# GiulioRomualdi/paper_romualdi_2022_icra_centroidal-mpc-walking

Hardware: AMD Instinct MI355X
Metric: centroidal-MPC solves/sec (batch, horizon=20) (higher is better)
Workload: dtype f32

## Files before the change

paper_romualdi_2022_icra_centroidal-mpc-walking_amd/csrc/cmpc_solver.hip:

```cpp
#include "cmpc_device.h"
#include "cmpc_launch.h"

#include <cstdlib>
#include <type_traits>
#include <map>
#include <mutex>

#define NS CMPC_NS
#define NF CMPC_NF
#define NQ CMPC_NQ
#define NU CMPC_NU
#define NXA CMPC_NXA
#define NI CMPC_NI
#define PLD 39
#define GLD 30
#define RLD 36
#define NPAN 46
#define GEO 36
#define SQ_TILE_WAVES 6
#define SQ_SPIN_MAX (1 << 20)
#define SQ_PUB_FLOATS (10 * NPAN * 4 + 128 * 4)
#define ZLD 36
#define MSET (NU * RLD + NPAN * RLD + NS * 16)
#define NTRI 256
// ... 1693 lines not shown
            if (ln < NU) Pann[(NPAN - 1) * RLD + ln] = (float)res;
            else if (ln < NU + NS) qsn[ln - NU] = res;
        } else {
            const bool two = wv == 3;
            v4f acc2 = {0.f, 0.f, 0.f, 0.f};
            CPROF(2);
#pragma unroll
            for (int b = 0; b < 8; b += 2) {
                float a0, b0, a1, b1;
                if (b == 6 && sk8 && sk9) {
                    need(7);
                    operands(6, a0, b0);
                    acc = __builtin_amdgcn_mfma_f32_16x16x4f32(a0, b0, acc, 0, 0, 0);
                    if (two) acc2 = __builtin_amdgcn_mfma_f32_16x16x4f32(a0, -a0, acc2, 0, 0, 0);
                    need(8);
                    operands(7, a1, b1);
                    acc = __builtin_amdgcn_mfma_f32_16x16x4f32(a1, b1, acc, 0, 0, 0);
                    if (two) acc2 = __builtin_amdgcn_mfma_f32_16x16x4f32(a1, -a1, acc2, 0, 0, 0);
                    continue;
                }
                need(b + 2);
                operands(b, a0, b0);
                operands(b + 1, a1, b1);
                acc = __builtin_amdgcn_mfma_f32_16x16x4f32(a0, b0, acc, 0, 0, 0);
                if (two) acc2 = __builtin_amdgcn_mfma_f32_16x16x4f32(a0, -a0, acc2, 0, 0, 0);
                acc = __builtin_amdgcn_mfma_f32_16x16x4f32(a1, b1, acc, 0, 0, 0);
                if (two) acc2 = __builtin_amdgcn_mfma_f32_16x16x4f32(a1, -a1, acc2, 0, 0, 0);
                if (b == 0) {
                    gaveup = !lds_wait_ge(c.flag + 3, SQ_TILE_WAVES * (ord + 1)) || gaveup;
                    acc += v4f{Mn[pl.d0], Mn[pl.d1], Mn[pl.d2], Mn[pl.d3]};
                    if (two) acc2 += v4f{Mn[pl.ri[5]], Mn[pl.ri[6]], Mn[pl.ri[7]], Mn[pl.ri[8]]};
                }
            }
            CPROF(3);
            if (!sk8 && !sk9) {
                float a0, b0, a1, b1;
                need(9);
                operands(8, a0, b0);
                acc = __builtin_amdgcn_mfma_f32_16x16x4f32(a0, b0, acc, 0, 0, 0);
                if (two) acc2 = __builtin_amdgcn_mfma_f32_16x16x4f32(a0, -a0, acc2, 0, 0, 0);
                need(10);
                operands(9, a1, b1);
                acc = __builtin_amdgcn_mfma_f32_16x16x4f32(a1, b1, acc, 0, 0, 0);
                if (two) acc2 = __builtin_amdgcn_mfma_f32_16x16x4f32(a1, -a1, acc2, 0, 0, 0);
            } else if (!sk8 || !sk9) {
                const int b = sk8 ? 9 : 8;
                need(b + 1);
                float a0, b0;
                operands(b, a0, b0);
                acc = __builtin_amdgcn_mfma_f32_16x16x4f32(a0, b0, acc, 0, 0, 0);
                if (two) acc2 = __builtin_amdgcn_mfma_f32_16x16x4f32(a0, -a0, acc2, 0, 0, 0);
            }
            CPROF2(4);
            {
                const float r0 = acc[0], r1 = acc[1], r2 = acc[2], r3 = acc[3];
                Mn[pl.d0] = r0; Mn[pl.d1] = r1; Mn[pl.d2] = r2; Mn[pl.d3] = r3;
                if (wv == 2 || wv == 4) { Mn[pl.ri[9]] = r0; Mn[pl.ri[10]] = r1; Mn[pl.ri[11]] = r2; Mn[pl.ri[12]] = r3; }
            }
            if (two) {
                const float r0 = acc2[0], r1 = acc2[1], r2 = acc2[2], r3 = acc2[3];
                Mn[pl.ri[5]] = r0; Mn[pl.ri[6]] = r1; Mn[pl.ri[7]] = r2; Mn[pl.ri[8]] = r3;
                Mn[pl.ri[9]] = r0; Mn[pl.ri[10]] = r1; Mn[pl.ri[11]] = r2; Mn[pl.ri[12]] = r3;
            }
        }
        CPROF(4);
    }
    if (gaveup && ln == 0) sq_give_up(c);
}
template <int NT, int NC, bool FG>
__device__ __attribute__((noinline)) void sq_consume_loop(lds_t lds, int Nrt, float* fg_base, int k0_in, bool exact_in, float reg, float cmu)
{
    CMPC_PHASE_PROLOGUE;
    const int k0 = __builtin_amdgcn_readfirstlane(k0_in);
    const bool use_exact = __builtin_amdgcn_readfirstlane((int)exact_in) != 0;
    ConsPlan pl;
    cons_plan_build(pl, c, prm, tid >> 6, tid & 63, c.Brow + ((N - 1) & 1) * DSET_I);
    sq_consume_stage(c, prm, pl, tid, N, N, N - 1, -1, 0, false, use_exact, reg, cmu);
    __syncthreads();
    int ord = 0;
#pragma unroll 1
    for (int k = N - 1; k >= k0; --k) {
        ++ord;
        if (k > k0) sq_consume_stage(c, prm, pl, tid, N, k, k - 1, k - 2 >= k0 ? k - 2 : -1, ord, true, use_exact, reg, cmu);
        __syncthreads();
    }
}
template <int NT, int NC, bool FG>
__device__ __attribute__((noinline)) void sq_init(lds_t lds, int Nrt, float* fg_base, int k0_in, bool exact_in, float cmu)
{
    CMPC_PHASE_PROLOGUE;
    const int k0 = __builtin_amdgcn_readfirstlane(k0_in);
    const bool use_exact = __builtin_amdgcn_readfirstlane((int)exact_in) != 0;
    {
        float* QN = c.Qb + (N & 1) * MSET;
        double* qN = (N & 1) ? c.qs1 : c.qs;
        if (tid < NS * 16) QN[tid] = (tid >> 4) == (tid & 15) ? qdiag(prm, N, tid & 15) : 0.f;
        else if (tid >= 256 && tid < 256 + NS) qN[tid - 256] = grad_track(c, prm, N, tid - 256);
        if (tid < 4) c.flag[tid] = 0;
        if (tid >= 128 && tid < 256) c.prog[tid - 128] = 0;
        if (tid >= 256 && tid < 256 + LATE_B * NLATE) {
            const int e = tid - 256, b = e / NLATE, r = e % NLATE;
            *reinterpret_cast<float4*>(c.ZT + (NPAN * b + NS + LATE_M0 + r) * 4) = make_float4(0.f, 0.f, 0.f, 0.f);
        }
    }
    if (tid >= 256) {
        const int kd = tid >= 384 ? N - 1 : N - 2;
        if (kd >= k0) {
            use_desc_set(c, kd & 1);
            stage_desc_body(c, prm, desc_pack_t(tid & 127), kd, use_exact, cmu);
        }
    }
    __syncthreads();
}
template <int NT, int NC, bool FG>
__device__ inline int riccati_backward_sq(lds_t lds, const Ctx& c, float* fg_base, bool use_exact, float reg, float cmu, int k0)
{
    const int N = c.N;
    sq_init<NT, NC, FG>(lds, N, fg_base, k0, use_exact, cmu);
    if (threadIdx.x < 64) sq_factor_loop<NT, NC, FG>(lds, N, fg_base, k0);
    else sq_consume_loop<NT, NC, FG>(lds, N, fg_base, k0, use_exact, reg, cmu);
    return (c.flag[0] ? 1 : 0) | (c.flag[1] ? 2 : 0);
}

template <int NT, int NC, bool FG>
__device__ int riccati_backward(lds_t lds, const Ctx& c, const CmpcConsts& prm, int tid, float* fg_base, bool use_exact, float reg, float cmu, int k0 = 0)
{
    if constexpr (!FG) return riccati_backward_sq<NT, NC, FG>(lds, c, fg_base, use_exact, reg, cmu, k0);
    const int N = c.N;
    for (int e = tid; e < NXA * PLD; e += NT) c.P0[e] = 0.f;
    if (tid == 0) *c.flag = 0;
    __syncthreads();
    if (tid < NS) {
        c.P0[tid * PLD + tid] = qdiag(prm, N, tid);
        c.pv[tid] = grad_track(c, prm, N, tid);
    } else if (tid < NXA) c.pv[tid] = 0.0;
    if (tid >= 128) stage_desc<NT, NC, FG>(lds, N, fg_base, N - 1, use_exact, cmu);
    __syncthreads();
    int tpk, tqp;
    {
        const int id0 = tid, id1 = tid + 128;
        tpk = (id0 < 135 ? c.tri[id0 / 3] : 0) | ((id1 < 135 ? c.tri[id1 / 3] : 0) << 16);
        const int tq = tid - 128, tile = tid;
        tqp = ((tq >= 0 && tq < 120) ? c.tri[tq] : 0) | ((tile < 210 ? c.tri[tile] : 0) << 16);
    }
    stage_pre<NT, NC, FG>(lds, N, fg_base, N - 1, false, use_exact, reg, cmu, tpk);
    for (int k = N - 1; k >= k0; --k) {
        if (((~__builtin_amdgcn_readfirstlane(c.qmask[k])) & 63) == 63) stage_mid<NT, NC, FG, true>(lds, N, fg_base, k, use_exact, cmu, tqp);
        else stage_mid<NT, NC, FG, false>(lds, N, fg_base, k, use_exact, cmu, tqp);
        if (k > k0 || k0 == 0) stage_post_pre<NT, NC, FG>(lds, N, fg_base, k, use_exact, reg, cmu, tpk, tqp);
    }
    return *c.flag ? 1 : 0;
}

template <int UNR, bool G>
__device__ __forceinline__ void forward_sweep(const Ctx& c, const CmpcConsts& prm, int tid, int k0)
{
    const int N = c.N;
    const int r = tid & 31, half = tid >> 5, blk = r >> 2;
    float* xb = c.ybuf;
    float* yb = c.ybuf + 40;
    float* trash = c.ybuf + 72;
    unsigned yoff[20], uoff[4];
#pragma unroll
    for (int t = 0; t < 20; ++t) {
        if (half == 0) yoff[t] = t < 16 ? wt_idx(t, r) : ub_row(t - 16) + r;
        else {
            const int m = 4 + t;
            yoff[t] = blk >= (m >> 2) ? ub_row(m) + r - 4 * (m >> 2) : REC_ZERO;
        }
    }
#pragma unroll
    for (int t = 0; t < 4; ++t) {
        const int q4 = 4 * half + t;
        uoff[t] = q4 >= blk ? ub_row(r) + 4 * (q4 - blk) : REC_ZERO;
    }
    const bool corner = tid < NF;
    const int ga = corner ? tid >> 3 : 0, cj = corner ? tid & 7 : 0;
    const int ga1 = (ga + 1) % 3, ga2 = (ga + 2) % 3;
    const int j = tid < NS ? tid : 0;
    const int ja = j % 3, ja1 = (ja + 1) % 3, ja2 = (ja + 2) % 3, jct = j >= 12 ? 1 : 0;
    const int je = j < 3 ? j + 3 : 0;
    const float ce = j < 3 ? prm.dt : 0.f;
    const float cD = (j >= 3 && j < 6) ? 1.f : 0.f, cH = (j >= 6 && j < 9) ? 1.f : 0.f;
    const float posm = j >= 9 ? 1.f : 0.f;
    const float cDm0 = ja == 0 ? cD : 0.f, cDm1 = ja == 1 ? cD : 0.f, cDm2 = ja == 2 ? cD : 0.f;
    const float cHm0 = ja == 0 ? cH : 0.f, cHm1 = ja == 1 ? cH : 0.f, cHm2 = ja == 2 ? cH : 0.f;
    const float gdtm = corner ? prm.dt : 0.f, gsel = cj >= 4 ? 1.f : 0.f, jsel = jct ? 1.f : 0.f;
    const float Dm = prm.D[r % 3];
    const float dtc = prm.dt;
    if (tid < 40) xb[tid] = tid == 15 ? 1.f : 0.f;
    if (tid < NS) c.dS[NS * k0 + tid] = 0.f;
    wave_lds_sync();
    ldsf_t yp[20];
    ldsf_t upp[4];
    if (!G) {
#pragma unroll
        for (int t = 0; t < 20; ++t) yp[t] = lds_opaque(c.Lf + (size_t)REC_N * k0 + yoff[t]);
#pragma unroll
        for (int t = 0; t < 4; ++t) upp[t] = lds_opaque(c.Lf + (size_t)REC_N * k0 + uoff[t]);
    }
    ldsf_t gr1 = lds_opaque(c.geoA + GEO * k0 + 3 * cj + ga1);
    ldsf_t gr2 = lds_opaque(c.geoA + GEO * k0 + 3 * cj + ga2);
    ldsf_t gf1 = lds_opaque(c.geoA + GEO * k0 + 24 + ja1);
    ldsf_t gf2 = lds_opaque(c.geoA + GEO * k0 + 24 + ja2);
    ldsf_t gm0 = lds_opaque(c.sp + c.L.pGam(0) + k0);
    ldsf_t gm1 = lds_opaque(c.sp + c.L.pGam(1) + k0);
    ldsf_t rp = lds_opaque(c.sp + c.L.pR(jct) + 9 * k0 + ja);
    ldsf_t dp = lds_opaque(c.d + NS * k0 + j);
    ldsf_t du0p = lds_opaque(c.dU + NU * k0 + 3 * cj + ga);
    ldsf_t du1p = lds_opaque(c.dU + NU * k0 + 3 * cj + ga1);
    ldsf_t du2p = lds_opaque(c.dU + NU * k0 + 3 * cj + ga2);
    ldsf_t dqp = lds_opaque(c.dU + NU * k0 + 24 + 3 * jct);
    ldsw_t dUs = lds_opaque_w(tid < NU ? c.dU + NU * k0 + tid : trash + (tid & 7));
    const int dUst = tid < NU ? NU : 0;
    ldsw_t dSs = lds_opaque_w(tid < NS ? c.dS + NS * (k0 + 1) + tid : trash + 8 + (tid & 7));
    const int dSst = tid < NS ? NS : 0;
    ldsw_t xbs = lds_opaque_w(tid < NS ? xb + tid : trash + 16 + (tid & 3));
    ldsw_t xps = lds_opaque_w(tid < NF ? xb + 16 + tid : trash + 20 + (tid & 3));
    ldsw_t ybs = lds_opaque_w(yb + r);
    ldsf_t xsp = lds_opaque(xb + j), xep = lds_opaque(xb + je), x1p = lds_opaque(xb + ja1), x2p = lds_opaque(xb + ja2);
    ldsf_t xvp = lds_opaque(xb + 20 * half), yvp = lds_opaque(yb + 16 * half);
    PROF2_DECL;
    float ymn[20];
    auto fetch = [&](int k) {
        const RecRef<G> rec(c.Lf, N, k);
#pragma unroll
        for (int t = 0; t < 20; ++t) ymn[t] = rec.ld(yoff[t]);
    };
    if (G) fetch(k0);
    auto stage = [&](int i, int k) {
        float ym[20];
        float4 um[4];
        if (G) {
            {
                const RecRef<G> rec(c.Lf, N, k);
#pragma unroll
                for (int t = 0; t < 4; ++t) um[t] = rec.ld4(uoff[t]);
            }
#pragma unroll
            for (int t = 0; t < 20; ++t) ym[t] = ymn[t];
            fetch(k + 1 < N ? k + 1 : k);
        } else {
#pragma unroll
            for (int t = 0; t < 20; ++t) ym[t] = yp[t][REC_N * i];
#pragma unroll
            for (int t = 0; t < 4; ++t) um[t] = lds_ld4(upp[t] + REC_N * i);
        }
        const float g_r1 = gr1[GEO * i], g_r2 = gr2[GEO * i];
        const float F01 = gf1[GEO * i], F11 = gf1[GEO * i + 3], F02 = gf2[GEO * i], F12 = gf2[GEO * i + 3];
        const float gam0 = gm0[i], gam1 = gm1[i];
        const float R0 = rp[9 * i], R1 = rp[9 * i + 3], R2 = rp[9 * i + 6];
        const float dk = dp[NS * i];
        const float dgam = gam1 - gam0;
        const float g_dt = gdtm * fmaf(gsel, dgam, gam0);
        const float gamj = fmaf(jsel, dgam, gam0);
        PROF2(20);
        float4 xv[5];
#pragma unroll
        for (int t = 0; t < 5; ++t) xv[t] = lds_ld4(xvp + 4 * t);
        float ya, yc;
        {
            v2f yp = v2f{ym[0], ym[1]} * v2f{xv[0].x, xv[0].y}, yq = v2f{ym[2], ym[3]} * v2f{xv[0].z, xv[0].w};
#pragma unroll
            for (int t = 1; t < 5; ++t) {
                yp = __builtin_elementwise_fma(v2f{ym[4 * t], ym[4 * t + 1]}, v2f{xv[t].x, xv[t].y}, yp);
                yq = __builtin_elementwise_fma(v2f{ym[4 * t + 2], ym[4 * t + 3]}, v2f{xv[t].z, xv[t].w}, yq);
            }
            yp += yq;
            ya = yp[0]; yc = yp[1];
        }
        const float y = half_sum(ya + yc);
        *ybs = y;
        wave_lds_sync();
        PROF2(21);
        float4 yv[4];
        if (G) {
#pragma unroll
            for (int q = 0; q < 4; ++q) yv[q] = lds_ld4(yvp + 4 * q);
        } else lds_ld4x4(yvp, yv);
        float wsum;
        {
            v2f wp = v2f{um[0].x, um[0].y} * v2f{yv[0].x, yv[0].y}, wq = v2f{um[0].z, um[0].w} * v2f{yv[0].z, yv[0].w};
#pragma unroll
            for (int q = 1; q < 4; ++q) {
                wp = __builtin_elementwise_fma(v2f{um[q].x, um[q].y}, v2f{yv[q].x, yv[q].y}, wp);
                wq = __builtin_elementwise_fma(v2f{um[q].z, um[q].w}, v2f{yv[q].z, yv[q].w}, wq);
            }
            wp += wq;
            wsum = wp[0] + wp[1];
        }
        const float du = -half_sum(wsum);
        *dUs = du;
        dUs += dUst;
        wave_lds_sync();
        PROF2(22);
        const float u0 = du0p[NU * i], u1 = du1p[NU * i], u2 = du2p[NU * i];
        const float xs = *xsp, xe = *xep;
        const float c1 = x1p[0], c2 = x2p[0];
        const float p01 = x1p[9], p02 = x2p[9], p11 = x1p[12], p12 = x2p[12];
        const float q0 = dqp[NU * i], q1 = dqp[NU * i + 1], q2 = dqp[NU * i + 2];
        const float tD = oct_sum(g_dt * u0);
        const float tH = oct_sum(g_dt * (g_r1 * u2 - g_r2 * u1));
        const float sDH = cDm0 * readlane_f(tD, 0) + cDm1 * readlane_f(tD, 8) + cDm2 * readlane_f(tD, 16)
                          + cHm0 * readlane_f(tH, 0) + cHm1 * readlane_f(tH, 8) + cHm2 * readlane_f(tH, 16);
        const float cross = gam0 * ((p01 - c1) * F02 - (p02 - c2) * F01) + gam1 * ((p11 - c1) * F12 - (p12 - c2) * F11);
        const float land = R0 * q0 + R1 * q1 + R2 * q2;
        const float out = fmaf(posm, gamj - 1.f, 1.f) * xs + ce * xe + sDH + cH * dtc * cross + dk + posm * (1.f - gamj) * land;
        wave_lds_sync();
        *dSs = out;
        dSs += dSst;
        *xbs = out;
        *xps = -Dm * du;
        wave_lds_sync();
        PROF2(23);
    };
    auto bump = [&](int n) {
        if (!G) {
#pragma unroll
            for (int t = 0; t < 20; ++t) yp[t] += REC_N * n;
#pragma unroll
            for (int t = 0; t < 4; ++t) upp[t] += REC_N * n;
#pragma unroll
            for (int t = 0; t < 20; ++t) asm volatile("" : "+v"(yp[t]));
#pragma unroll
            for (int t = 0; t < 4; ++t) asm volatile("" : "+v"(upp[t]));
        }
        gr1 += GEO * n; gr2 += GEO * n; gf1 += GEO * n; gf2 += GEO * n; gm0 += n; gm1 += n; rp += 9 * n; dp += NS * n;
        du0p += NU * n; du1p += NU * n; du2p += NU * n; dqp += NU * n;
    };
    int k = k0;
#pragma unroll 1
    for (; k + UNR <= N; k += UNR) {
#pragma unroll
        for (int i = 0; i < UNR; ++i) stage(i, k + i);
        bump(UNR);
    }
#pragma unroll 1
    for (; k < N; ++k) {
        stage(0, k);
        bump(1);
    }
}
template <int NT, int UNR, bool G, int PART = 0>
__device__ void riccati_forward(const Ctx& c, const CmpcConsts& prm, int tid, bool affine, int k0)
{
    const int N = c.N;
    if (PART != 2 && tid < 64) forward_sweep<UNR, G>(c, prm, tid, k0);
    if (PART == 1) return;
    __syncthreads();
    for (int e = tid + NI * k0; e < N * NI; e += NT) {
        const int k = e / NI, i = e % NI;
        float dt_ = 0.f, dz_ = 0.f;
        if (row_active(c, k, i)) {
            const float t = c.T[e], z = c.Z[e];
            const float cmu = affine ? 0.f : c.dZ[e];
            const float r = row_val(c, prm, k, i, c.U + NU * k) + t;
            dt_ = -r - row_dot(c, prm, k, i, c.dU + NU * k);
            dz_ = (cmu - z * t) / t - (z / t) * dt_;
        }
        c.dT[e] = dt_; c.dZ[e] = dz_;
    }
    __syncthreads();
}

template <int UNR, bool G>
__device__ __forceinline__ void delta_sweep(const Ctx& c, const CmpcConsts& prm, int tid)
{
    const int N = c.N;
    const int r = tid & 31, half = tid >> 5, blk = r >> 2;
    float* gb = c.ybuf;
    float* lb = c.ybuf + 32;
    float* trash = c.ybuf + 72;
    unsigned loff[16], foff[8];
#pragma unroll
// ... 260 lines not shown
    const float t1 = readlane_f(v, 16), t2 = readlane_f(v, 32), t3 = readlane_f(v, 48);
    const int row = lane >> 4;
    return v + (row == 0 ? t1 + (t2 + t3) : (row == 1 ? t2 + t3 : (row == 2 ? t3 : 0.f)));
}
__device__ inline float suffix_lin(float g, float b, int lane)
{
#define CMPC_LIN_STEP(CT) { const float gn = dpp_keep<CT>(1.f, g), bn = dpp_f<CT>(b); b = fmaf(g, bn, b); g *= gn; }
    CMPC_LIN_STEP(0x101) CMPC_LIN_STEP(0x102) CMPC_LIN_STEP(0x104) CMPC_LIN_STEP(0x108)
#undef CMPC_LIN_STEP
    const int row = lane >> 4;
    const float v48 = readlane_f(b, 48);
    if (row == 2) b = fmaf(g, v48, b);
    const float v32 = readlane_f(b, 32);
    if (row == 1) b = fmaf(g, v32, b);
    const float v16 = readlane_f(b, 16);
    if (row == 0) b = fmaf(g, v16, b);
    return b;
}
__device__ __forceinline__ float costate_com_b(float w, float err, float egm, float dtm, float dF1, float dF2, float lo1, float lo2, float vh1, float vh2, float g1,
                                               float g2)
{
    float b = w * err;
    b += egm * (dF2 * lo1 - dF1 * lo2);
    b += dtm * (vh1 * g2 - vh2 * g1);
    return b;
}
__device__ __forceinline__ float costate_foot_b(float w, float err, float egm, float dtm, float gam, float dF1, float dF2, float lo1, float lo2, float vh1, float vh2,
                                                float g1, float g2)
{
    float b = w * err;
    b += egm * (dF1 * lo2 - dF2 * lo1);
    b -= dtm * gam * (vh1 * g2 - vh2 * g1);
    return b;
}
__device__ __forceinline__ float sel3(const float (&v)[3], int i) { return i == 0 ? v[0] : (i == 1 ? v[1] : v[2]); }
__device__ inline void costate_scan_axis(const Ctx& c, const CmpcConsts& prm, int lane, int ax, bool use_exact, float* vout)
{
    const int N = c.N;
    const bool valid = lane <= N, dyn = lane < N;
    const int k = valid ? lane : N, kd = dyn ? lane : N - 1;
    const int a1 = ax == 2 ? 0 : ax + 1, a2 = ax == 0 ? 2 : ax - 1;
    const float* S = c.S + NS * k;
    const float* dS = c.dS + NS * k;
    const float* geo = c.geoA + GEO * kd;
    const float* du = c.dU + NU * kd;
    const float* lo = c.LAM + NS * (kd + 1) + 6;
    const float dtm = dyn ? prm.dt : 0.f;
    const float egm = use_exact ? dtm : 0.f;
    const float on = valid ? 1.f : 0.f;
    const float gam0 = gam_of(c, 0, kd), gam1 = gam_of(c, 1, kd);
    float dF1[3], dF2[3];
    dF1[0] = gam0 * (du[a1] + du[3 + a1] + du[6 + a1] + du[9 + a1]);
    dF1[1] = gam1 * (du[12 + a1] + du[15 + a1] + du[18 + a1] + du[21 + a1]);
    dF1[2] = dF1[0] + dF1[1];
    dF2[0] = gam0 * (du[a2] + du[3 + a2] + du[6 + a2] + du[9 + a2]);
    dF2[1] = gam1 * (du[12 + a2] + du[15 + a2] + du[18 + a2] + du[21 + a2]);
    dF2[2] = dF2[0] + dF2[1];
    const float lo1 = lo[a1], lo2 = lo[a2];
    float vh[3], vhn[3];
#pragma unroll
    for (int a = 0; a < 3; ++a) {
        const float b = on * (2.f * prm.w_h) * ((S[6 + a] - c.sp[c.L.pHref() + a + 3 * k]) + dS[6 + a]);
        vh[a] = suffix_sum(b, lane);
    }
#pragma unroll
    for (int a = 0; a < 3; ++a) vhn[a] = lane_next(vh[a], lane);
    const float vh1 = sel3(vhn, a1), vh2 = sel3(vhn, a2);
    const float w = ax == 0 ? 2.f * prm.w_com0 : (ax == 1 ? 2.f * prm.w_com1 : prm.wz2[k]);
    const float bc = costate_com_b(w, (S[ax] - c.sp[c.L.pComref() + ax + 3 * k]) + dS[ax], egm, dtm, dF1[2], dF2[2], lo1, lo2, vh1, vh2, geo[30 + a1], geo[30 + a2]);
    const float vc = suffix_sum(on * bc, lane);
    float vf[2];
#pragma unroll
    for (int ct = 0; ct < 2; ++ct) {
        const float gam = ct ? gam1 : gam0;
        const int j = 9 + 3 * ct + ax;
        const float b = costate_foot_b(2.f * prm.w_pos, (S[j] - c.sp[c.L.pNom(ct) + ax + 3 * k]) + dS[j], egm, dtm, gam, dF1[ct], dF2[ct], lo1, lo2, vh1, vh2,
                                       geo[24 + 3 * ct + a1], geo[24 + 3 * ct + a2]);
        vf[ct] = suffix_lin(dyn ? gam : 1.f, on * b, lane);
    }
    const float vv = suffix_sum(dtm * lane_next(vc, lane), lane);
    if (valid && lane > 0) {
        float* o = vout + NS * k + ax;
        o[0] = vc; o[3] = vv; o[6] = sel3(vh, ax); o[9] = vf[0]; o[12] = vf[1];
    }
}
template <bool DEFER>
__device__ inline void costate_scan(const Ctx& c, const CmpcConsts& prm, int lane, float ap, bool use_exact, float* vout)
{
    const int N = c.N;
    const bool valid = lane <= N, dyn = lane < N;
    const int k = valid ? lane : N, kd = dyn ? lane : N - 1;
    const float* S = c.S + NS * k;
    const float* dS = c.dS + NS * k;
    const float* geo = c.geoA + GEO * kd;
    const float* dF = c.d + NS * kd;
    const float dtm = dyn ? prm.dt : 0.f;
    const float egm = use_exact ? dtm : 0.f;
    const float on = valid ? 1.f : 0.f;
    float lo[3];
#pragma unroll
    for (int a = 0; a < 3; ++a) lo[a] = c.LAM[NS * (kd + 1) + 6 + a];
    float lold[NS];
    if (!DEFER) {
#pragma unroll
        for (int j = 0; j < NS; ++j) lold[j] = c.LAM[NS * k + j];
    }
    float v[NS];
    float vh1[3];
#pragma unroll
    for (int a = 0; a < 3; ++a) {
        const float b = on * (2.f * prm.w_h) * ((S[6 + a] - c.sp[c.L.pHref() + a + 3 * k]) + dS[6 + a]);
        v[6 + a] = suffix_sum(b, lane);
    }
#pragma unroll
    for (int a = 0; a < 3; ++a) vh1[a] = lane_next(v[6 + a], lane);
#pragma unroll
    for (int a = 0; a < 3; ++a) {
        const int a1 = (a + 1) % 3, a2 = (a + 2) % 3;
        const float w = a == 0 ? 2.f * prm.w_com0 : (a == 1 ? 2.f * prm.w_com1 : prm.wz2[k]);
        const float b = costate_com_b(w, (S[a] - c.sp[c.L.pComref() + a + 3 * k]) + dS[a], egm, dtm, dF[6 + a1], dF[6 + a2], lo[a1], lo[a2], vh1[a1], vh1[a2],
                                      geo[30 + a1], geo[30 + a2]);
        v[a] = suffix_sum(on * b, lane);
    }
#pragma unroll
    for (int ct = 0; ct < 2; ++ct) {
        const float gam = c.sp[c.L.pGam(ct) + kd];
#pragma unroll
        for (int a = 0; a < 3; ++a) {
            const int a1 = (a + 1) % 3, a2 = (a + 2) % 3, j = 9 + 3 * ct + a;
            const float b = costate_foot_b(2.f * prm.w_pos, (S[j] - c.sp[c.L.pNom(ct) + a + 3 * k]) + dS[j], egm, dtm, gam, dF[3 * ct + a1], dF[3 * ct + a2], lo[a1],
                                           lo[a2], vh1[a1], vh1[a2], geo[24 + 3 * ct + a1], geo[24 + 3 * ct + a2]);
            v[j] = suffix_lin(dyn ? gam : 1.f, on * b, lane);
        }
    }
#pragma unroll
    for (int a = 0; a < 3; ++a) v[3 + a] = suffix_sum(dtm * lane_next(v[a], lane), lane);
    if (valid && lane > 0) {
#pragma unroll
        for (int j = 0; j < NS; ++j) {
            if (DEFER) vout[NS * k + j] = v[j];
            else c.LAM[NS * k + j] = lold[j] + ap * (v[j] - lold[j]);
        }
    }
}

__device__ void costate_update(const Ctx& c, const CmpcConsts& prm, int tid, float ap, bool use_exact)
{
    costate_force_sums(c, tid, blockDim.x);
    __syncthreads();
    if (tid < 64) costate_scan<false>(c, prm, tid, ap, use_exact, nullptr);
    __syncthreads();
}

template <int NT, int NC, bool FG, int PART>
__device__ __attribute__((noinline)) void phase_forward_part(lds_t lds, int Nrt, float* fg_base, bool affine_in)
{
    CMPC_PHASE_PROLOGUE;
    const bool affine = __builtin_amdgcn_readfirstlane((int)affine_in) != 0;
    riccati_forward<NT, NC == 0 ? 1 : (FG ? 2 : SWEEP_UNROLL), FG, PART>(c, prm, tid, affine, 0);
}
template <int NT, int NC, bool FG>
__device__ __forceinline__ void phase_forward_sweep(lds_t lds, int Nrt, float* fg_base, bool affine_in)
{
    if (threadIdx.x < 64) phase_forward_part<NT, NC, FG, 1>(lds, Nrt, fg_base, affine_in);
}
template <int NT, int NC, bool FG>
__device__ __attribute__((noinline)) void phase_forward_tail(lds_t lds, int Nrt, float* fg_base, bool affine_in, int k0_in)
{
    CMPC_PHASE_PROLOGUE;
    const bool affine = __builtin_amdgcn_readfirstlane((int)affine_in) != 0;
    const int k0 = __builtin_amdgcn_readfirstlane(k0_in);
    riccati_forward<NT, 1, FG>(c, prm, tid, affine, k0);
}
template <int NT, int NC, bool FG>
__device__ __attribute__((noinline)) void phase_delta_part(lds_t lds, int Nrt, float* fg_base)
{
    CMPC_PHASE_PROLOGUE;
    riccati_delta<NC == 0 ? 1 : (FG ? 2 : DELTA_UNROLL), FG>(c, prm, tid);
}
template <int NT, int NC, bool FG>
__device__ __forceinline__ void phase_delta(lds_t lds, int Nrt, float* fg_base)
{
    if (threadIdx.x < 64) phase_delta_part<NT, NC, FG>(lds, Nrt, fg_base);
    __syncthreads();
}
template <int NT, int NC, bool FG>
__device__ __attribute__((noinline)) void phase_costate(lds_t lds, int Nrt, float* fg_base, float ap, bool exact_in)
{
    CMPC_PHASE_PROLOGUE;
    const bool use_exact = __builtin_amdgcn_readfirstlane((int)exact_in) != 0;
    costate_update(c, prm, tid, ap, use_exact);
}
__device__ inline float dual_extrapolate(float z, float dz) { return fmaxf(z + dz, 0.f); }

template <int NT, int NC, bool FG>
__device__ __attribute__((noinline)) void tail_polish(lds_t lds, int Nrt, float* fg_base, int k0_in, bool duals_in)
{
    CMPC_PHASE_PROLOGUE;
    const int k0 = __builtin_amdgcn_readfirstlane(k0_in);
    const bool duals = __builtin_amdgcn_readfirstlane((int)duals_in) != 0;
    bool last = false, blocked = true;
    for (int pi = 0; pi <= prm.tail_iters + 6 && !last; ++pi) {
        last = pi >= prm.tail_iters + 6 || (pi >= prm.tail_iters && !blocked);
        all_geo<NT>(c, prm, tid);
        for (int e = tid + NS * k0; e < NS * N; e += NT) c.d[e] = (float)defect(c, prm, e / NS, e % NS);
        __syncthreads();
        const float cmu = last ? 0.f : -prm.mu_min;
        int fail = riccati_backward<NT, NC, FG>(lds, c, prm, tid, fg_base, prm.exact_hessian != 0, prm.reg, cmu, k0);
        if (fail) {
            __syncthreads();
            fail = riccati_backward<NT, NC, FG>(lds, c, prm, tid, fg_base, false, prm.reg, cmu, k0);
        }
        if (fail) break;
        if (!last) {
            for (int e = tid + NI * k0; e < NI * N; e += NT) c.dZ[e] = row_active(c, e / NI, e % NI) ? row_target(c.Z[e], prm.mu_min) : 0.f;
            __syncthreads();
        }
        phase_forward_tail<NT, NC, FG>(lds, N, fg_base, last, k0);
        float ap, ad;
        step_lengths<NT>(c, tid, last ? 0.999f : 0.99f, ap, ad, k0);
        float bad = 0.f;
        for (int e = tid + NU * k0; e < NU * N; e += NT) bad = amax_nan(bad, c.dU[e]);
        for (int e = tid + NS * (k0 + 1); e < NS * (N + 1); e += NT) bad = amax_nan(bad, c.dS[e]);
        float m1[1] = {bad};
        block_maxn<NT, 1>(m1, c.red, tid);
        if (!(m1[0] < INFINITY)) break;
        blocked = ap < 0.9f || ad < 0.9f;
        for (int e = tid + NS * (k0 + 1); e < NS * (N + 1); e += NT) c.S[e] += ap * c.dS[e];
        for (int e = tid + NU * k0; e < NU * N; e += NT) c.U[e] += ap * c.dU[e];
        if (!last)
            for (int e = tid + NI * k0; e < NI * N; e += NT) { c.T[e] += ap * c.dT[e]; c.Z[e] += ad * c.dZ[e]; }
        else if (duals)
            for (int e = tid + NI * k0; e < NI * N; e += NT) {
                const float tn = c.T[e] + ap * c.dT[e], zn = dual_extrapolate(c.Z[e], c.dZ[e]);
                if (fabsf(tn) < INFINITY && fabsf(zn) < INFINITY) { c.T[e] = tn; c.Z[e] = zn; }
            }
        __syncthreads();
    }
}

struct Resid { float ep, ec, mu; };
template <int NT, int NC, bool FG>
constexpr bool kLeanPasses = NT == 512 && NC > 0 && !FG;
template <int NT, int NC, bool FG>
__device__ __attribute__((noinline)) Resid phase_residuals(lds_t lds, int Nrt, float* fg_base, int nrow_in)
{
    CMPC_PHASE_PROLOGUE;
    const int nrow = __builtin_amdgcn_readfirstlane(nrow_in);
    float l_ep = 0.f, l_ec = 0.f, l_chk = 0.f;
    double l_mu = 0.0;
    all_geo<NT>(c, prm, tid);
    for (int e = tid; e < 24 * N; e += NT) {
        const int k = e / 24, r = e - 24 * k, a = r >> 3, cj = r & 7, ct = cj >> 2;
        const int a1 = (a + 1) % 3, a2 = (a + 2) % 3;
        const float* s = c.S + NS * k;
        const float* f = c.U + NU * k + 3 * cj;
        const float* R = c.sp + c.L.pR(ct) + 9 * k;
        const float* cn = prm.corners + 3 * cj;
        const double r1 = (double)Rm(R, a1, 0) * cn[0] + (double)Rm(R, a1, 1) * cn[1] + (double)Rm(R, a1, 2) * cn[2] + (double)s[9 + 3 * ct + a1] - (double)s[a1];
        const double r2 = (double)Rm(R, a2, 0) * cn[0] + (double)Rm(R, a2, 1) * cn[1] + (double)Rm(R, a2, 2) * cn[2] + (double)s[9 + 3 * ct + a2] - (double)s[a2];
        double t = (double)gam_of(c, ct, k) * (r1 * (double)f[a2] - r2 * (double)f[a1]);
        t += dpp_d<0xB1>(t);
        t += dpp_d<0x4E>(t);
        t += dpp_d<0x141>(t);
        if (cj == 0) {
            const double dv = (double)s[6 + a] + (double)prm.dt * ((double)c.sp[c.L.pText() + 3 * k + a] + t) - (double)c.S[NS * (k + 1) + 6 + a];
            c.d[NS * k + 6 + a] = (float)dv;
            l_ep = fmaxf(l_ep, fabsf((float)dv));
            l_chk += (float)dv;
        }
    }
    constexpr int LGRP = (3 * NC + 63) / 64 * 64;
    if constexpr (NC > 0 && !FG && 4 * LGRP <= NT) {
        static_assert((LGRP & (LGRP - 1)) == 0, "the lane inside a group is taken with a mask");
        const int tl = tid - (NT - 4 * LGRP);
        const int grp = __builtin_amdgcn_readfirstlane(tl >= 0 ? tl / LGRP : -1);
        const int l = tl & (LGRP - 1);
        if (grp >= 0 && l < 3 * NC) {
            const int a = (l >= NC ? 1 : 0) + (l >= 2 * NC ? 1 : 0), k = l - NC * a;
            double dv;
            int i;
            if (grp == 0) { i = a; dv = defect_com(c, prm, k, a); }
            else if (grp == 1) { i = 3 + a; dv = defect_vel(c, prm, k, a); }
            else { i = 9 + 3 * (grp - 2) + a; dv = defect_foot(c, prm, k, grp - 2, a); }
            c.d[NS * k + i] = (float)dv;
            l_ep = fmaxf(l_ep, fabsf((float)dv));
            l_chk += (float)dv;
        }
    } else {
        for (int e = tid; e < 12 * N; e += NT) {
            const int k = e / 12, ii = e - 12 * k, i = ii < 6 ? ii : ii + 3;
            const double dv = ii < 3 ? defect_com(c, prm, k, ii) : (ii < 6 ? defect_vel(c, prm, k, ii - 3) : defect_foot(c, prm, k, ii < 9 ? 0 : 1, ii < 9 ? ii - 6 : ii - 9));
            c.d[NS * k + i] = (float)dv;
            l_ep = fmaxf(l_ep, fabsf((float)dv));
            l_chk += (float)dv;
        }
    }
    if constexpr (NC > 0) {
        for_slots<0, RowSlots<NT, NC>::R>([&](auto qc) {
            constexpr int q = decltype(qc)::value;
            int e;
            float val, dot;
            const int st = row_slot<NT, NC, q, false>(c, prm, tid, e, val, dot);
            const float t = c.T[e], z = c.Z[e];
            if (st & 2) {
                const float rv = val + t;
                l_ep = fmaxf(l_ep, fabsf(rv));
                l_ec = fmaxf(l_ec, t * z);
                l_chk += rv + t * z;
                l_mu += (double)t * z;
            }
        });
    } else {
        for (int e = tid; e < NI * N; e += NT) {
            const int k = e / NI, i = e % NI;
            if (row_active(c, k, i)) {
                const float t = c.T[e], z = c.Z[e];
                const float rv = row_val(c, prm, k, i, c.U + NU * k) + t;
                l_ep = fmaxf(l_ep, fabsf(rv));
                l_ec = fmaxf(l_ec, t * z);
                l_chk += rv + t * z;
                l_mu += (double)t * z;
            }
        }
    }
    if (!(fabsf(l_chk) < INFINITY)) l_ep = INFINITY;
    block_max2_sum<NT, !kLeanPasses<NT, NC, FG>>(l_ep, l_ec, l_mu, c.red, c.redd, tid);
    Resid r;
    r.ep = l_ep; r.ec = l_ec; r.mu = (float)(l_mu / (double)nrow);
    return r;
}

template <int NT, int NC, bool FG>
__device__ __attribute__((noinline)) float phase_update(lds_t lds, int Nrt, float* fg_base, float ap_in, float ad_in)
{
    CMPC_PHASE_PROLOGUE;
    const float ap = uniform_f(ap_in), ad = uniform_f(ad_in);
    for (int e = tid; e < NS * (N + 1); e += NT) c.S[e] += ap * c.dS[e];
    for (int e = tid; e < NU * N; e += NT) c.U[e] += ap * c.dU[e];
    for (int e = tid; e < NI * N; e += NT) {
        const float tn = c.T[e] + ap * c.dT[e];
        float zn = c.Z[e] + ad * c.dZ[e];
        c.T[e] = tn; c.Z[e] = zn;
    }
    float l_st = 0.f, l_sf = 0.f, l_fm = 1.f, l_chk2 = 0.f;
    for (int e = tid; e < NS * (N + 1); e += NT) { const float ds = c.dS[e]; l_st = fmaxf(l_st, fabsf(ds)); l_chk2 += ds; }
    for (int e = tid; e < NU * N; e += NT) {
        const int k = e / NU, m = e % NU;
        const float du = c.dU[e];
        l_chk2 += du;
        if (m < NF) {
            const float* f = c.dU + NU * k + 12 * (m / 12) + m % 3;
            const float mean = 0.25f * (f[0] + f[3] + f[6] + f[9]);
            l_sf = fmaxf(l_sf, fabsf(du - gam_of(c, m / 12, k) * mean));
            if (k > 0) l_sf = fmaxf(l_sf, fabsf(du - c.dU[e - NU]));
            l_fm = fmaxf(l_fm, fabsf(c.U[e]));
        } else l_st = fmaxf(l_st, fabsf(du));
    }
    if (!(fabsf(l_chk2) < INFINITY)) l_st = INFINITY;
    float m3[3] = {l_st, l_sf, l_fm};
    block_maxn<NT, 3>(m3, c.red, tid);
    return ap * fmaxf(m3[0], m3[1] / m3[2]);
}

template <int NT, int NC, bool FG>
__device__ __attribute__((noinline)) bool phase_finish(lds_t lds, int Nrt, float* fg_base, bool duals_in)
{
    CMPC_PHASE_PROLOGUE;
    const bool duals = __builtin_amdgcn_readfirstlane((int)duals_in) != 0;
    float ap, ad;
    step_lengths<NT>(c, tid, 0.999f, ap, ad);
    const int kt = N - prm.tail_stages;
    float l_all = 0.f, l_tail = 0.f, l_fm = 1.f;
    for (int e = tid; e < NS * (N + 1); e += NT) l_all = amax_nan(l_all, c.dS[e]);
    for (int e = tid; e < NU * N; e += NT) {
        const float du = c.dU[e];
        l_all = amax_nan(l_all, du);
        if (e % NU < NF) {
            l_fm = fmaxf(l_fm, fabsf(c.U[e]));
            if (e >= NU * kt) l_tail = fmaxf(l_tail, fabsf(du));
        }
    }
    float m3[3] = {l_all, l_tail, l_fm};
    block_maxn<NT, 3>(m3, c.red, tid);
    if (!(m3[0] < INFINITY)) return false;
    const int k0 = (prm.tail_stages > 0 && m3[1] > prm.tail_trigger * m3[2]) ? kt : N;
    if (k0 < N) step_lengths<NT>(c, tid, 0.999f, ap, ad, 0, k0);
    for (int e = tid; e < NS * (k0 < N ? k0 + 1 : N + 1); e += NT) c.S[e] += ap * c.dS[e];
    for (int e = tid; e < NU * k0; e += NT) c.U[e] += ap * c.dU[e];
    if (duals)
        for (int e = tid; e < NI * k0; e += NT) {
            const float tn = c.T[e] + ap * c.dT[e], zn = dual_extrapolate(c.Z[e], c.dZ[e]);
            if (fabsf(tn) < INFINITY && fabsf(zn) < INFINITY) { c.T[e] = tn; c.Z[e] = zn; }
        }
    __syncthreads();
    if (k0 == N) return false;
// ... 271 lines not shown
        const float du = c.dU[e];
        l_chk2 += du;
        if (mm < NF) {
            const float* f = c.dU + NU * k + 12 * (mm / 12) + mm % 3;
            const float mean = 0.25f * (f[0] + f[3] + f[6] + f[9]);
            l_sf = fmaxf(l_sf, fabsf(du - gam_of(c, mm / 12, k) * mean));
            if (k > 0) l_sf = fmaxf(l_sf, fabsf(du - c.dU[e - NU]));
            l_fm = fmaxf(l_fm, fabsf(c.U[e]));
        } else l_st = fmaxf(l_st, fabsf(du));
    }
    if (!(fabsf(l_chk2) < INFINITY)) l_st = INFINITY;
    float m3[3] = {l_st, l_sf, l_fm};
    block_maxn<NT, 3, !LEAN>(m3, LEAN ? c.red1 : c.red, tid);
    FinalStep r;
    r.ap = ap; r.ad = ad; r.step = ap * fmaxf(m3[0], m3[1] / m3[2]);
    return r;
}

template <int NT, int NC, bool FG>
__device__ __attribute__((noinline)) void phase_export(lds_t lds, int Nrt, float* fg_base, float* x, float* dq, int status_in)
{
    CMPC_PHASE_PROLOGUE;
    for (int e = tid; e < NS * (N + 1); e += NT) {
        const int k = e / NS, i = e % NS;
        if (i < 9) x[c.L.oCom() + 3 * (N + 1) * (i / 3) + 3 * k + i % 3] = c.S[e];
        else x[c.L.oPos((i - 9) / 3) + 3 * k + (i - 9) % 3] = c.S[e];
    }
    for (int e = tid; e < NU * N; e += NT) {
        const int k = e / NU, m = e % NU;
        if (m < NF) x[c.L.oF(m / 12, (m % 12) / 3) + 3 * k + m % 3] = c.U[e];
        else {
            const int q = m - 24, ct = q / 3, i = q % 3;
            const float v = gam_of(c, ct, k) < 0.5f ? (c.S[NS * (k + 1) + 9 + q] - c.S[NS * k + 9 + q]) / prm.dt : 0.f;
            x[c.L.oVel(ct) + 3 * k + i] = v;
        }
    }
    if (dq) {
        const int status = __builtin_amdgcn_readfirstlane(status_in);
        __syncthreads();
        if (status != 3) {
            all_geo<NT>(c, prm, tid);
            for (int e = tid; e < NS * (N + 1); e += NT) c.dS[e] = 0.f;
            for (int e = tid; e < NS * N; e += NT) c.d[e] = 0.f;
            __syncthreads();
            if (tid < 64) costate_scan<true>(c, prm, tid, 0.f, false, c.LAM);
            __syncthreads();
        }
        for (int e = tid; e < NS * (N + 1); e += NT) dq[e] = e < NS ? (e == 0 ? (float)status : 0.f) : c.LAM[e];
        for (int e = tid; e < NI * N; e += NT) { dq[NS * (N + 1) + e] = c.T[e]; dq[NS * (N + 1) + NI * N + e] = c.Z[e]; }
    }
#ifdef CMPC_PROFILE
    if (prm.hwid_probe) {
        __syncthreads();
        if ((threadIdx.x & 63) == 0) x[threadIdx.x >> 6] = (float)(__builtin_amdgcn_s_getreg((31 << 11) | 4) & 0xffff);
    }
#endif
}

template <int NT, int NC, bool FG>
__global__ __launch_bounds__(NT, FG ? 3 : 1) void cmpc_solve_kernel(CmpcParams kp)
{
    extern __shared__ __attribute__((aligned(16))) char smem[];
    const int b = blockIdx.x;
    if (kp.ended && kp.ended[b] >= 0) return;
    const bool fresh = kp.start && kp.start[b] == kp.tick;
    const bool warm = kp.warm && !fresh;
    const float mu_init0 = fresh ? kp.cold_mu_init : kp.mu_init, t_floor0 = fresh ? kp.cold_t_floor : kp.t_floor, mu_adapt0 = fresh ? kp.cold_mu_adapt : kp.mu_adapt;
    const int tid = threadIdx.x;
    const int N = NC > 0 ? NC : kp.N;
    {
        int* z = reinterpret_cast<int*>(smem);
        for (int e = tid; e < kp.lds_words; e += NT) z[e] = 0;
    }
    __syncthreads();
    {
        const int* src = reinterpret_cast<const int*>(kp.kc_per_problem ? kp.kc + b : kp.kc);
        int* dst = reinterpret_cast<int*>(smem);
        for (int e = tid; e < (int)(sizeof(CmpcConsts) / 4); e += NT) dst[e] = src[e];
    }
    const CmpcConsts& prm = *reinterpret_cast<const CmpcConsts*>(smem);
    const long long t_start = __builtin_amdgcn_s_memtime();
    unsigned ldsv = (unsigned)(unsigned long long)(lds_t)smem;
    asm volatile("" : "+s"(ldsv));
    const lds_t lds = (lds_t)(unsigned long long)ldsv;
    float* const fg_base = FG ? kp.scratch + (size_t)b * kp.scratch_stride : nullptr;
    const CmpcIdx L{N};
    __syncthreads();
    const bool outside = (phase_setup<NT, NC, FG>(lds, N, fg_base, kp.P + (size_t)b * L.np()) != 0) | (prm.model_bad != 0);
    int status = 1, sg = 0, it_total = 0;
    float err = 0.f, ep = 0.f, mu_cur = 0.f, step_out = 0.f, step_prev = 0.f;
    float* const dq = kp.duals ? kp.duals + (size_t)b * (NS * (N + 1) + 2 * NI * N) : nullptr;
    if (outside) {
        phase_init<NT, NC, FG>(lds, N, fg_base, kp.X0 + (size_t)b * L.nx(), dq, 0, mu_init0, t_floor0);
        status = 3;
    }
    for (int pass = 0; pass < 2 && !outside; ++pass) {
        const float mu_init = pass ? 0.1f : mu_init0, t_floor = pass ? 1e-2f : t_floor0, mu_adapt = pass ? 3.5f : mu_adapt0;
        step_out = step_prev = 0.f;
        const bool use_duals = warm && kp.warm_duals && kp.duals;
        const int nrow = phase_init<NT, NC, FG>(lds, N, fg_base, kp.X0 + (size_t)b * L.nx(), dq,
                                                (pass > 0 ? 1 : 0) | (use_duals ? 2 : 0) | (use_duals && kp.warm_duals > 1 ? 4 : 0), mu_init, t_floor);
        int it = 0;
        status = 1;
        bool finishing = false;
        const int budget = (warm && pass == 0 && kp.warm_budget > 0 && kp.warm_budget < prm.max_iter) ? kp.warm_budget : prm.max_iter;
        for (it = 0; it < budget + 1; ++it) {
            if (it == budget && !finishing) break;
            PROF_DECL;
            const Resid rs = phase_residuals<NT, NC, FG>(lds, N, fg_base, nrow);
            ep = rs.ep;
            const float ec = rs.ec;
            mu_cur = rs.mu;
            if (!(ep < INFINITY)) { status = 2; err = INFINITY; break; }
            if (it == 0 && mu_adapt > 0.f) {
                const float mu0 = fminf(fmaxf(mu_adapt * ep * ep, 0.03f), 0.5f);
                phase_multipliers<NT, NC, FG>(lds, N, fg_base, 0, mu0 / mu_cur, nrow);
                mu_cur = mu0;
            }
            if (warm && pass == 0 && it > 0 && ec > 100.f * mu_cur && ec > 0.1f) {
                mu_cur = phase_multipliers<NT, NC, FG>(lds, N, fg_base, 1, mu_cur, nrow);
                sg += 100;
            }
            PROF(10);
            float est = step_out;
            if (it > 1 && step_prev > 0.f) {
                const float rho = fminf(fmaxf(step_out / step_prev, 0.2f), 0.9f);
                est = fminf(est, step_out * rho / (1.f - rho));
            }
            if (it > 0 && !finishing && fmaxf(ep, ec) <= prm.tol && est <= prm.step_tol) {
                err = fmaxf(ep, ec);
                status = 0;
                if (!prm.final_extrap) break;
                finishing = true;
            }
            const bool centring = !finishing && mu_cur <= fmaxf(1.5f * prm.mu_min, 0.15f * prm.tol) && ec <= fmaxf(4.f * prm.mu_min, 0.4f * prm.tol);
            bool exact = prm.exact_hessian != 0;
            float reg = prm.reg;
            int fail = 1;
            bool resync = false;
            for (int attempt = 0; attempt < 4; ++attempt) {
                fail = phase_backward<NT, NC, FG>(lds, N, fg_base, exact, reg, centring ? prm.mu_min : 0.f);
                if (!fail) break;
                __syncthreads();
                if (fail & 2) {
                    sg += 1000000;
                    if (!resync) { resync = true; --attempt; continue; }
                }
                ++sg; exact = false;
                if (attempt > 0) reg *= 1e3f;
            }
            if (fail) { if (!finishing) status = 2; break; }
            PROF(11);
            float sigma = 0.f, mu_t = prm.mu_min;
            if (centring) {
                phase_multipliers<NT, NC, FG>(lds, N, fg_base, 2, prm.mu_min, nrow);
            } else {
                phase_forward_sweep<NT, NC, FG>(lds, N, fg_base, true);
                PROF(12);
                if (finishing) {
                    phase_forward_part<NT, NC, FG, 2>(lds, N, fg_base, true);
                    if (phase_finish<NT, NC, FG>(lds, N, fg_base, dq != nullptr)) sg += 100000;
                    ++it;
                    break;
                }
                Centre ce;
                if constexpr (NC > 0) ce = phase_affine_post<NT, NC, FG>(lds, N, fg_base, mu_cur, nrow);
                else {
                    phase_forward_part<NT, NC, FG, 2>(lds, N, fg_base, true);
                    const StepLen sa = phase_step_lengths<NT, NC, FG>(lds, N, fg_base, 1.f);
                    ce = phase_corrector_targets<NT, NC, FG>(lds, N, fg_base, sa.ap, sa.ad, mu_cur, nrow);
                }
                sigma = ce.sigma; mu_t = ce.mu_t;
                PROF(13);
                phase_delta<NT, NC, FG>(lds, N, fg_base);
                PROF(14);
            }
            phase_forward_sweep<NT, NC, FG>(lds, N, fg_base, false);
            PROF(15);
            float ap, ad, step;
            if constexpr (NC > 0) {
                const FinalStep fs = phase_final_post<NT, NC, FG>(lds, N, fg_base, fmaxf(0.99f, 1.f - mu_t), exact);
                ap = fs.ap; ad = fs.ad; step = fs.step;
                PROF(16);
            } else {
                phase_forward_part<NT, NC, FG, 2>(lds, N, fg_base, false);
                const StepLen sl = phase_step_lengths<NT, NC, FG>(lds, N, fg_base, fmaxf(0.99f, 1.f - mu_t));
                ap = sl.ap; ad = sl.ad;
                phase_costate<NT, NC, FG>(lds, N, fg_base, ap, exact);
                PROF(16);
                step = phase_update<NT, NC, FG>(lds, N, fg_base, ap, ad);
            }
            step_prev = step_out;
            step_out = step;
            err = fmaxf(ep, ec);
    #ifdef CMPC_PROFILE
            if (tid == 0 && b == 0 && it < 64) {
                float* tr = g_trace + 8 * it;
                tr[0] = mu_cur; tr[1] = ep; tr[2] = ec; tr[3] = step; tr[4] = ap; tr[5] = ad; tr[6] = sigma; tr[7] = mu_t;
            }
    #endif
            PROF(17);
            if (err <= prm.tol && step <= prm.step_tol) {
                status = 0;
                if (!prm.final_extrap) { ++it; break; }
                finishing = true;
            }
        }
        it_total += it;
        if (status == 0 || !warm || pass > 0 || kp.warm_no_restart) break;
        sg += 10000;
        __syncthreads();
    }
    phase_export<NT, NC, FG>(lds, N, fg_base, kp.X + (size_t)b * L.nx(), dq, status);
    if (kp.info && tid == 0) {
        float* inf = kp.info + (size_t)b * CMPC_INFO_N;
        inf[0] = (float)it_total; inf[1] = err; inf[2] = mu_cur; inf[3] = (float)sg; inf[4] = ep; inf[5] = (float)status;
        inf[6] = (float)(__builtin_amdgcn_s_memtime() - t_start); inf[7] = step_out;
    }
}

}

extern "C" size_t cmpc_solver_lds_bytes(int N, int factors_global)
{
    CmpcLayout L;
    cmpc_layout_init(L, N);
    const size_t dbl = 90 + 40 + 40 + 16 + 40 + 4 * NI + 8 + (factors_global ? 0 : 90 + 16);
    const size_t work = factors_global ? ((NXA * PLD + 3) & ~3) + NS * 16 + ((NXA * GLD + 3) & ~3) : (size_t)MSET + NS * 16 + SQ_PUB_FLOATS + 128;
    const size_t flt = (size_t)NU * RLD + (size_t)NPAN * RLD + 96 + ID_STRIPS + ((L.np + 3) & ~3)
                       + ((size_t)NS * (N + 1) + (size_t)NU * N + ((factors_global && N > CMPC_TZ_LDS_NMAX) ? 0 : 2 * (size_t)NI * N)) + (size_t)NS * N + (size_t)NS * (N + 1)
                       + (size_t)GEO * N + work + 2 * DSET_F + 40 + 40 + 24
                       + 2 * DSET_I + 4 + CMPC_NMAX + NTRI / 2 + (factors_global ? 0 : (size_t)REC_N * N);
    return ((sizeof(CmpcConsts) + 15) & ~(size_t)15) + dbl * 8 + flt * 4;
}

#ifdef CMPC_PROFILE
extern "C" int cmpc_profile_read(long long* out, int reset)
{
    hipError_t e = hipMemcpyFromSymbol(out, HIP_SYMBOL(g_prof), sizeof(long long) * 128);
    if (reset) { long long z[128] = {0}; (void)hipMemcpyToSymbol(HIP_SYMBOL(g_prof), z, sizeof(z)); }
    return (int)e;
}
extern "C" int cmpc_trace_read(float* out) { return (int)hipMemcpyFromSymbol(out, HIP_SYMBOL(g_trace), sizeof(float) * 64 * 8); }
#endif

typedef void (*cmpc_kernel_t)(CmpcParams);
static cmpc_kernel_t solver_variant(int N, bool factors_global, int& nthreads)
{
    constexpr int NT = 256, NR = 512;
    if (factors_global) {
        nthreads = NT;
        return N == 20 ? cmpc_solve_kernel<NT, 20, true> : (N == 30 ? cmpc_solve_kernel<NT, 30, true> : cmpc_solve_kernel<NT, 0, true>);
    }
    nthreads = NR;
    switch (N) {
        case 10: return cmpc_solve_kernel<NR, 10, false>;
        case 12: return cmpc_solve_kernel<NR, 12, false>;
        case 13: return cmpc_solve_kernel<NR, 13, false>;
        case 15: return cmpc_solve_kernel<NR, 15, false>;
        case 20: return cmpc_solve_kernel<NR, 20, false>;
        case 22: return cmpc_solve_kernel<NR, 22, false>;
        default: return cmpc_solve_kernel<NR, 0, false>;
    }
}
extern "C" int cmpc_prepare_solver(int N, int factors_global, size_t lds_bytes)
{
    int nthreads = 0;
    const cmpc_kernel_t kern = solver_variant(N, factors_global != 0, nthreads);
    int dev = 0;
    if (hipGetDevice(&dev) != hipSuccess) dev = 0;
    static std::mutex mu;
    static std::map<std::pair<int, const void*>, size_t> limit;
    std::lock_guard<std::mutex> lock(mu);
    size_t& cur = limit[std::make_pair(dev, reinterpret_cast<const void*>(kern))];
    if (lds_bytes <= cur) return 0;
    const hipError_t e = hipFuncSetAttribute(reinterpret_cast<const void*>(kern), hipFuncAttributeMaxDynamicSharedMemorySize, (int)lds_bytes);
    if (e == hipSuccess) cur = lds_bytes;
    return (int)e;
}
extern "C" int cmpc_launch_solver(const CmpcParams* prm, size_t lds_bytes, hipStream_t stream)
{
    int nthreads = 0;
    const cmpc_kernel_t kern = solver_variant(prm->N, prm->scratch != nullptr, nthreads);
    CmpcParams kp = *prm;
    kp.lds_words = (int)(lds_bytes / 4);
    (void)hipGetLastError();
    hipLaunchKernelGGL(kern, dim3(prm->B), dim3(nthreads), lds_bytes, stream, kp);
    return (int)hipGetLastError();
}
```

Measured before the change: 379,400.

## Overlap forward-sweep setup with delta phase via wave handoff

For the lean 512-thread configuration, the delta phase now runs on wave 0 while wave 2 starts the forward sweep early. It loads its loop-invariant LDS pointers and constants before waiting on a block barrier, then initialises its buffers and sweeps. This hides the sweep prologue latency behind the delta computation and removes one extra barrier. The cost is more complex barrier pairing across waves: every wave must reach matching __syncthreads calls, which makes deadlocks or ordering bugs possible.

```diff
diff --git a/paper_romualdi_2022_icra_centroidal-mpc-walking_amd/csrc/cmpc_solver.hip b/paper_romualdi_2022_icra_centroidal-mpc-walking_amd/csrc/cmpc_solver.hip
--- a/paper_romualdi_2022_icra_centroidal-mpc-walking_amd/csrc/cmpc_solver.hip
+++ b/paper_romualdi_2022_icra_centroidal-mpc-walking_amd/csrc/cmpc_solver.hip
@@ -1869,9 +1869,11 @@
     return *c.flag ? 1 : 0;
 }
 
-template <int UNR, bool G>
-__device__ __forceinline__ void forward_sweep(const Ctx& c, const CmpcConsts& prm, int tid, int k0)
-{
+struct NoGate { __device__ __forceinline__ void operator()() const {} };
+template <int UNR, bool G, class GATE = NoGate>
+__device__ __forceinline__ void forward_sweep(const Ctx& c, const CmpcConsts& prm, int tid, int k0, GATE gate = GATE())
+{
+    constexpr bool GATED = !std::is_same<GATE, NoGate>::value;
     const int N = c.N;
     const int r = tid & 31, half = tid >> 5, blk = r >> 2;
     float* xb = c.ybuf;
@@ -1905,9 +1907,11 @@
     const float gdtm = corner ? prm.dt : 0.f, gsel = cj >= 4 ? 1.f : 0.f, jsel = jct ? 1.f : 0.f;
     const float Dm = prm.D[r % 3];
     const float dtc = prm.dt;
-    if (tid < 40) xb[tid] = tid == 15 ? 1.f : 0.f;
-    if (tid < NS) c.dS[NS * k0 + tid] = 0.f;
-    wave_lds_sync();
+    if constexpr (!GATED) {
+        if (tid < 40) xb[tid] = tid == 15 ? 1.f : 0.f;
+        if (tid < NS) c.dS[NS * k0 + tid] = 0.f;
+        wave_lds_sync();
+    }
     ldsf_t yp[20];
     ldsf_t upp[4];
     if (!G) {
@@ -1937,6 +1941,12 @@
     ldsw_t ybs = lds_opaque_w(yb + r);
     ldsf_t xsp = lds_opaque(xb + j), xep = lds_opaque(xb + je), x1p = lds_opaque(xb + ja1), x2p = lds_opaque(xb + ja2);
     ldsf_t xvp = lds_opaque(xb + 20 * half), yvp = lds_opaque(yb + 16 * half);
+    if constexpr (GATED) {
+        gate();
+        if (tid < 40) xb[tid] = tid == 15 ? 1.f : 0.f;
+        if (tid < NS) c.dS[NS * k0 + tid] = 0.f;
+        wave_lds_sync();
+    }
     PROF2_DECL;
     float ymn[20];
     auto fetch = [&](int k) {
@@ -2503,12 +2513,21 @@
     __syncthreads();
 }
 
+template <int NT, int NC, bool FG>
+constexpr bool kLeanPasses = NT == 512 && NC > 0 && !FG;
+template <int NT, int NC, bool FG>
+constexpr bool kSweepHandoff = kLeanPasses<NT, NC, FG>;
 template <int NT, int NC, bool FG, int PART>
-__device__ __attribute__((noinline)) void phase_forward_part(lds_t lds, int Nrt, float* fg_base, bool affine_in)
+__device__ __attribute__((noinline)) void phase_forward_part(lds_t lds, int Nrt, float* fg_base, bool affine_in, bool gate_in = false)
 {
     CMPC_PHASE_PROLOGUE;
-    const bool affine = __builtin_amdgcn_readfirstlane((int)affine_in) != 0;
-    riccati_forward<NT, NC == 0 ? 1 : (FG ? 2 : SWEEP_UNROLL), FG, PART>(c, prm, tid, affine, 0);
+    if constexpr (PART == 1 && kSweepHandoff<NT, NC, FG>) {
+        const bool gated = __builtin_amdgcn_readfirstlane((int)gate_in) != 0;
+        forward_sweep<SWEEP_UNROLL, false>(c, prm, tid & 63, 0, [&] { if (gated) __syncthreads(); });
+    } else {
+        const bool affine = __builtin_amdgcn_readfirstlane((int)affine_in) != 0;
+        riccati_forward<NT, NC == 0 ? 1 : (FG ? 2 : SWEEP_UNROLL), FG, PART>(c, prm, tid, affine, 0);
+    }
 }
 template <int NT, int NC, bool FG>
 __device__ __forceinline__ void phase_forward_sweep(lds_t lds, int Nrt, float* fg_base, bool affine_in)
@@ -2591,8 +2610,6 @@
 }
 
 struct Resid { float ep, ec, mu; };
-template <int NT, int NC, bool FG>
-constexpr bool kLeanPasses = NT == 512 && NC > 0 && !FG;
 template <int NT, int NC, bool FG>
 __device__ __attribute__((noinline)) Resid phase_residuals(lds_t lds, int Nrt, float* fg_base, int nrow_in)
 {
@@ -3170,6 +3187,7 @@
             if (fail) { if (!finishing) status = 2; break; }
             PROF(11);
             float sigma = 0.f, mu_t = prm.mu_min;
+            [[maybe_unused]] const int wv = __builtin_amdgcn_readfirstlane(tid >> 6);
             if (centring) {
                 phase_multipliers<NT, NC, FG>(lds, N, fg_base, 2, prm.mu_min, nrow);
             } else {
@@ -3190,10 +3208,20 @@
                 }
                 sigma = ce.sigma; mu_t = ce.mu_t;
                 PROF(13);
-                phase_delta<NT, NC, FG>(lds, N, fg_base);
-                PROF(14);
-            }
-            phase_forward_sweep<NT, NC, FG>(lds, N, fg_base, false);
+                if constexpr (!kSweepHandoff<NT, NC, FG>) {
+                    phase_delta<NT, NC, FG>(lds, N, fg_base);
+                    PROF(14);
+                } else if (wv == 0) phase_delta_part<NT, NC, FG>(lds, N, fg_base);
+            }
+            if constexpr (kSweepHandoff<NT, NC, FG>) {
+                if (wv == 2) phase_forward_part<NT, NC, FG, 1>(lds, N, fg_base, false, true);
+                else __syncthreads();
+#ifdef CMPC_PROFILE
+                if (!centring) PROF(14);
+                __syncthreads();
+#endif
+            } else
+                phase_forward_sweep<NT, NC, FG>(lds, N, fg_base, false);
             PROF(15);
             float ap, ad, step;
             if constexpr (NC > 0) {
```

After: 382,000 (median of 6 runs). Within noise of the previous version (+0.7%).
